# jessegrabowski/gEconpy

Hardware: AMD Instinct MI355X
Metric: solve+Kalman-logp evals/sec, Smets-Wouters n~40 T=200 (higher is better)
Workload: dtype f64; 1 GPU; sw_shaped synthetic (SURVEY 8d): n=m=40, n_state=18, n_lead=12, k=7, p=7, T_len=200, 4096 draws per GPU (BASELINE configs[2]); global_batch=4096, solver=cycle_reduction, inputs=A,B,C,D resident in HBM, parallelism=single GPU

## Files before the change

### geconpy_amd/csrc/dsge_kalman_mf.hpp

```cpp
#pragma once
#include <type_traits>

#include "dsge_kalman_nt.hpp"
#include "dsge_kalman_rec.hpp"
#include "dsge_mfma4.hpp"

namespace dsge {

template <int KT, int TM>
struct KmfSmem {
  static_assert(KT >= 1 && KT <= TM && TM <= 8, "tiles");
  static constexpr int NS = 4 * KT, NM = 4 * TM;
  static constexpr int LDK = NS + 2;
  static constexpr int NR = 8 * ((NM + 7) / 8);
  static constexpr int RP = NR / 8, PS = 10;
  static constexpr int WT = NM * LDK > NR * PS ? NM * LDK : NR * PS;
  static constexpr size_t doubles = (size_t)NM * LDK + WT + (size_t)NS * LDK + 2 * (size_t)NR * PS + 2 * NR + 4 + 44 + NR / 2 + 4;
  static constexpr size_t bytes = sizeof(double) * doubles;
};

#ifndef KMF_WAVES
#define KMF_WAVES 2
#endif
template <int KT, int TM, bool DBG, bool REC = false, int RBS = (4 * TM + 7) / 8>
__global__ __launch_bounds__(64, KMF_WAVES) void kalman_mf_kernel(
    const double* __restrict__ T, const double* __restrict__ RQR, const double* __restrict__ P0, const double* __restrict__ Z,
    int z_batched, const double* __restrict__ dvec, int d_batched, const double* __restrict__ Hdiag, int h_batched,
    const double* __restrict__ y, int batch, int m_full, int p, int T_len, FilterConv cv, double missing_fill, double steady_tol,
    double* __restrict__ logp_out, int32_t* __restrict__ status, long long* __restrict__ dbg, int rerun_only,
    int32_t* __restrict__ steady_at, const int32_t* __restrict__ order, const double* __restrict__ Rsel,
    const double* __restrict__ qdiag, int q_batched, int k_shocks, const unsigned long long* __restrict__ colmask_in,
    double* __restrict__ rec_store = nullptr) {
  using SM = KmfSmem<KT, TM>;
  using RC = KgRec<RBS>;
  static_assert(!REC || (4 * TM <= 8 * RBS && Mfma4Upper<TM>::NG * 64 <= 8 * RBS * 8 * RBS), "the record's tile holds the filter's");
  using UX = Mfma4Upper<TM>;
  using MW = Mfma4Map<KT, TM>;
  constexpr int NS = SM::NS, NM = SM::NM, LDK = SM::LDK, NR = SM::NR, RP = SM::RP, PS = SM::PS, NG = UX::NG;
  constexpr bool LEAN = NG > 5;
  extern __shared__ __attribute__((aligned(16))) double smem[];
  double* Tc = smem;
  double* Wt = Tc + NM * LDK;
  double* Vs = Wt;
  double* Pc = Wt + SM::WT;
  double* PZt = Pc + NS * LDK;
  double* Ks = PZt + NR * PS;
  double* av = Ks + NR * PS;
  double* avd = av;
  double* af = av + NR + 2;
  double* vv = af + NR + 2;
  double* dd = vv + 10;
  double* hh = dd + 8;
  double* zv = hh + 8;
  double* zvt = zv + 8;
  int* perm = (int*)(zvt + 10);
  int* zpos = perm + NR;
  constexpr int W_DUMP = (NM - 1) * LDK + LDK - 1;
  constexpr int TC_DUMP = (NM - 1) * LDK + LDK - 1;
  constexpr int PC_DUMP = (NS - 1) * LDK + LDK - 1;
  constexpr int PZ_DUMP = (NR - 1) * PS + PS - 1;
  const int lane = threadIdx.x;
  const int blk = (lane >> 2) & 3, i4 = lane & 3, kq = lane >> 4;
  const double LN2PI = 1.8378770664093453, LN2 = 0.6931471805599453;

  if (rerun_only && rerun_pass_is_empty(status, batch, order)) return;
  for (int bi = blockIdx.x; bi < batch; bi = batch) {
    const int draw = __builtin_amdgcn_readfirstlane(order ? order[bi] : bi);
    const int32_t st_in = __builtin_amdgcn_readfirstlane(status[draw]);
    if (rerun_only) {
      if (st_in != DSGE_ST_INTERNAL_RERUN) continue;
    } else if (st_in != 0) {
      if (lane == 0) logp_out[draw] = -INFINITY;
      continue;
    }
    const size_t off = (size_t)draw * m_full * m_full;
    wave_sync();
    for (int idx = lane; idx < (int)SM::doubles; idx += 64) smem[idx] = 0.0;

    const double* Zg = Z + (z_batched ? (size_t)draw * p * m_full : 0);
    bool is_state = false;
    const unsigned long long cm_in = colmask_in ? colmask_in[draw] : ~0ull;
    if (cm_in != ~0ull) {
      is_state = (lane < m_full) && ((cm_in >> lane) & 1ull);
    } else {
      const double* tcol = T + off + (lane < m_full ? lane : 0);
      for (int r0 = 0; r0 < m_full; r0 += 8) {
        double tv[8];
#pragma unroll
        for (int u = 0; u < 8; ++u) tv[u] = tcol[(size_t)(r0 + u < m_full ? r0 + u : m_full - 1) * m_full];
        __builtin_amdgcn_sched_barrier(0);
#pragma unroll
        for (int u = 0; u < 8; ++u) is_state |= (tv[u] != 0.0);
      }
      is_state = is_state && (lane < m_full);
    }
    const unsigned long long colmask = __ballot(is_state);
    unsigned long long obsmask = 0ull, used = 0ull;
    bool ok = true;
    double zrow[8];
    {
      const int zl_lane = lane < m_full ? lane : m_full - 1;
#pragma unroll
      for (int o = 0; o < 8; ++o) zrow[o] = Zg[(size_t)(o < p ? o : (p > 0 ? p - 1 : 0)) * m_full + zl_lane];
      __builtin_amdgcn_sched_barrier(0);
#pragma unroll
      for (int o = 0; o < 8; ++o) zrow[o] = (lane < m_full && o < p) ? zrow[o] : 0.0;
    }
#pragma unroll
    for (int o = 0; o < 8; ++o) {
      if (o < p) {
        const unsigned long long b = __ballot(zrow[o] != 0.0);
        if (__popcll(b) != 1 || ((used & b) != 0ull)) ok = false;
        used |= b;
        obsmask |= b;
      }
    }
    const unsigned long long extra = obsmask & ~colmask;
    const int s = __popcll(colmask);
    const int m = s + __popcll(extra);
    ok = ok && (s <= NS) && (m <= NM) && (s >= 1);
    int my_pos = -1;
    if (lane < m_full) {
      const unsigned long long below = (1ull << lane) - 1ull;
      if ((colmask >> lane) & 1ull)
        my_pos = __popcll(colmask & below);
      else if ((extra >> lane) & 1ull)
        my_pos = s + __popcll(extra & below);
      if (my_pos >= 0 && my_pos < NR) perm[my_pos] = lane;
    }
#pragma unroll
    for (int o = 0; o < 8; ++o) {
      if (o < p && zrow[o] != 0.0) {
        zpos[o] = (my_pos >= 0 && my_pos < NR) ? my_pos : 0;
        zv[o] = zrow[o];
      }
    }
    if (!ok) {
      if (lane == 0) status[draw] = DSGE_ST_INTERNAL_RERUN;
      continue;
    }
    if (rerun_only && lane == 0) status[draw] = 0;
    wave_sync();

    int rr[NG], cc[NG];
    bool inm[NG], up[NG];
    constexpr int NT_ = LEAN ? 1 : NG;
    int pcw0_[NT_], pcw1_[NT_];
    int pzw0[NG], pzw1[NG];
    double pzv0_[NT_], pzv1_[NT_];
    if (lane < 9) zvt[lane] = (lane < p) ? zv[lane] : 0.0;
#pragma unroll
    for (int g = 0; g < NG; ++g) {
      int ta, tb;
      bool live;
      UX::tile(g, blk, ta, tb, live);
      const int r = 4 * ta + kq, c = 4 * tb + i4;
      rr[g] = r;
      cc[g] = c;
      inm[g] = live && r < m && c < m;
      up[g] = live && r <= c;
      int oc = -1, orr = -1;
      double zc = 0.0, zr = 0.0;
      for (int o = 0; o < p; ++o) {
        if (zpos[o] == c) {
          oc = o;
          zc = zv[o];
        }
        if (zpos[o] == r) {
          orr = o;
          zr = zv[o];
        }
      }
      const bool w0 = up[g] && inm[g] && oc >= 0, w1 = up[g] && inm[g] && r < c && orr >= 0;
      if constexpr (LEAN) {
        pzw0[g] = ((w0 ? r * PS + oc : PZ_DUMP) << 4) | (w0 ? oc : 8);
        pzw1[g] = ((w1 ? c * PS + orr : PZ_DUMP) << 4) | (w1 ? orr : 8);
      } else {
        const bool in_pc = up[g] && c < NS;
        pcw0_[g] = in_pc ? r * LDK + c : PC_DUMP;
        pcw1_[g] = (in_pc && r < c) ? c * LDK + r : PC_DUMP;
        pzw0[g] = w0 ? r * PS + oc : PZ_DUMP;
        pzw1[g] = w1 ? c * PS + orr : PZ_DUMP;
        pzv0_[g] = zc;
        pzv1_[g] = zr;
      }
    }
    int rowa[NG], rowb[NG];
    mfma4_upper_rows<TM>(lane, rowa, rowb);
    auto pcw0 = [&](int g) {
      if constexpr (LEAN) return (up[g] && cc[g] < NS) ? rr[g] * LDK + cc[g] : PC_DUMP;
      else return pcw0_[g];
    };
    auto pcw1 = [&](int g) {
      if constexpr (LEAN) return (up[g] && cc[g] < NS && rr[g] < cc[g]) ? cc[g] * LDK + rr[g] : PC_DUMP;
      else return pcw1_[g];
    };
    wave_sync();

    auto load_T = [&]() {
      lane_loop_batched<8>(m * s, lane,
                           [&](int idx) {
                             const int r = idx / s, c = idx - r * s;
                             return T[off + (size_t)perm[r] * m_full + perm[c]];
                           },
                           [&](int idx, double v) {
                             const int r = idx / s, c = idx - r * s;
                             Tc[r * LDK + c] = v;
                           });
    };
    double Qt[NG], Pt[NG];
    if (Rsel) {
      const int kp = (k_shocks + 1) & ~1;
      const double* Rg = Rsel + (size_t)draw * m_full * k_shocks;
      for (int idx = lane; idx < m_full * k_shocks; idx += 64) {
        const int i = idx / k_shocks, c = idx - i * k_shocks;
        Wt[i * kp + c] = Rg[idx];
      }
      const double* qd = qdiag + (q_batched ? (size_t)draw * k_shocks : 0);
      wave_sync();
#pragma unroll
      for (int g = 0; g < NG; ++g) {
        const double2* ri = reinterpret_cast<const double2*>(Wt + (inm[g] ? perm[rr[g]] : 0) * kp);
        const double2* rj = reinterpret_cast<const double2*>(Wt + (inm[g] ? perm[cc[g]] : 0) * kp);
        double a0 = 0.0, a1 = 0.0;
        for (int c2 = 0; 2 * c2 < kp; ++c2) {
          const double2 ti = ri[c2], tj = rj[c2];
          a0 = fma(ti.x * tj.x, qd[2 * c2], a0);
          a1 = fma(ti.y * tj.y, (2 * c2 + 1 < k_shocks) ? qd[2 * c2 + 1] : 0.0, a1);
        }
        Qt[g] = inm[g] ? a0 + a1 : 0.0;
      }
      wave_sync();
      for (int idx = lane; idx < m_full * kp; idx += 64) Wt[idx] = 0.0;
    } else {
#pragma unroll
      for (int g = 0; g < NG; ++g) Qt[g] = inm[g] ? RQR[off + (size_t)perm[rr[g]] * m_full + perm[cc[g]]] : 0.0;
    }
#pragma unroll
    for (int g = 0; g < NG; ++g) Pt[g] = (inm[g] && P0) ? P0[off + (size_t)perm[rr[g]] * m_full + perm[cc[g]]] : 0.0;
    load_T();
    wave_sync();
#define KMF_STORE_PC()                        \
  do {                                        \
    _Pragma("unroll") for (int g = 0; g < NG; ++g) { \
      Pc[pcw0(g)] = Pt[g];                    \
      Pc[pcw1(g)] = Pt[g];                    \
    }                                         \
  } while (0)
    if (!P0) {
#pragma unroll
      for (int g = 0; g < NG; ++g) Pt[g] = Qt[g];
      bool lyap_ok = false;
      for (int itl = 0; itl < 64; ++itl) {
        wave_sync();
        KMF_STORE_PC();
        wave_sync();
        mfma4_nt<KT, KT, TM, LDK>(Pc, Tc, lane, [&](int g, double d) {
          const int at = (4 * MW::tb(g, blk) + i4) * LDK + 4 * MW::ta(g, blk) + kq;
          Wt[MW::live(g, blk) ? at : W_DUMP] = d;
        });
        using MA = Mfma4Map<TM, KT>;
        double a2r[MA::NG];
        mfma4_nn<KT, TM, KT, LDK>(Tc, Tc, lane, [&](int g, double d) { a2r[g] = d; });
        wave_sync();
        double dmax = 0.0, pmax = 0.0;
        mfma4_nt_upper_acc<KT, TM, LDK>(Tc, Wt, lane, rowa, rowb, [](int) { return 0.0; }, [&](int g, double d) {
          const double dlt = inm[g] ? d : 0.0;
          Pt[g] += dlt;
          dmax = nanmax(dmax, fabs(dlt));
          pmax = nanmax(pmax, fabs(Pt[g]));
        });
        wave_sync();
#pragma unroll
        for (int g = 0; g < MA::NG; ++g) {
          const int at = (4 * MA::ta(g, blk) + kq) * LDK + 4 * MA::tb(g, blk) + i4;
          Tc[MA::live(g, blk) ? at : TC_DUMP] = a2r[g];
        }
        dmax = wave_nanmax(dmax);
        pmax = wave_nanmax(pmax);
        if (!(dmax == dmax) || !(pmax < 1e300)) break;
        if (dmax <= 1e-17 * pmax) {
          lyap_ok = true;
          break;
        }
      }
      wave_sync();
      for (int idx = lane; idx < NM * LDK; idx += 64) Tc[idx] = 0.0;
      for (int idx = lane; idx < SM::WT; idx += 64) Wt[idx] = 0.0;
      wave_sync();
      load_T();
      if (!lyap_ok) {
        if (lane == 0) {
          status[draw] |= DSGE_ST_LYAP_FAIL;
          logp_out[draw] = -INFINITY;
        }
        continue;
      }
    }
    double* const rec_d = REC ? rec_store + (size_t)draw * RC::per_draw(T_len) : nullptr;
    int seg_src = -1;
    if constexpr (REC) {
      constexpr int RNP = 8 * RBS;
      double* p0s = rec_d + (size_t)T_len * RC::STEP;
      for (int idx = lane; idx < RNP * RNP; idx += 64) {
        const int r = idx / RNP, c = idx - r * RNP;
        if (!(r < m && c < m)) p0s[idx] = 0.0;
      }
#pragma unroll
      for (int g = 0; g < NG; ++g) {
        if (up[g] && inm[g]) {
          p0s[rr[g] * RNP + cc[g]] = Pt[g];
          p0s[cc[g] * RNP + rr[g]] = Pt[g];
        }
      }
      if (lane == 0) rec_d[RC::tail_state_off(T_len) + RC::TS_LAYOUT] = (double)(RC::LAYOUT_TILES + TM);
    }
    if (lane < 8) {
      dd[lane] = (dvec && lane < p) ? dvec[(d_batched ? (size_t)draw * p : 0) + lane] : 0.0;
      hh[lane] = (Hdiag && lane < p) ? Hdiag[(h_batched ? (size_t)draw * p : 0) + lane] : 0.0;
    }
#define KMF_STORE_PZT()                                 \
  do {                                                  \
    _Pragma("unroll") for (int g = 0; g < NG; ++g) {    \
      if constexpr (LEAN) {                             \
        PZt[pzw0[g] >> 4] = zvt[pzw0[g] & 15] * Pt[g];  \
        PZt[pzw1[g] >> 4] = zvt[pzw1[g] & 15] * Pt[g];  \
      } else {                                          \
        PZt[pzw0[g]] = pzv0_[g] * Pt[g];                \
        PZt[pzw1[g]] = pzv1_[g] * Pt[g];                \
      }                                                 \
    }                                                   \
  } while (0)
    KMF_STORE_PZT();
    const int v_zpos = (lane < p) ? zpos[lane] : 0;
    const double v_zv = (lane < p) ? zv[lane] : 0.0, v_dd = (lane < 8) ? dd[lane & 7] : 0.0;
    wave_sync();

    const int r8 = lane & 7, g8 = lane >> 3;
    const int r_zpos = (r8 < p) ? zpos[r8] : 0;
    const double r_zv = (r8 < p) ? zv[r8] : 0.0, r_dd = dd[r8], r_hh = hh[r8];
    const bool fold_a = m < NM;

    double quad_sum = 0.0, quad_comp = 0.0;
    double ld_mant = 1.0;
    int ld_exp = 0;
    int n_ll_steps = 0, n_obs_entries = 0;
    long long ph[8] = {0, 0, 0, 0, 0, 0, 0, 0};
    const long long tk_start = DBG ? clock64() : 0;
    int steady_step = -1;
    const int r8c = (r8 < p) ? r8 : (p > 0 ? p - 1 : 0);
    double yt_next = (T_len > 0) ? y[r8c] : 0.0;
    for (int t = 0; t < T_len; ++t) {
      long long tk0 = DBG ? clock64() : 0;
      const double yt = yt_next;
      yt_next = y[(size_t)((t + 1 < T_len) ? t + 1 : t) * p + r8c];
      const bool obs = (r8 < p) && (yt == yt) && (yt != missing_fill);
      const unsigned long long omask = __ballot(obs) & 0xffull;
      const int n_obs = __popcll(omask);
      double* const sg = REC ? rec_d + (size_t)t * RC::STEP : nullptr;
      if constexpr (REC) {
        if (lane < 8 * RBS) sg[RC::OFF_A + lane] = (lane < NR) ? av[lane] : 0.0;
        if (lane == 0) {
          sg[RC::OFF_SRC] = (double)t;
          sg[RC::OFF_PREV] = (double)seg_src;
        }
        seg_src = t;
      }
      double2 fr2[4], pz2[RP][4];
      double pzo[RP], avi[RP];
#pragma unroll
      for (int q2 = 0; q2 < 4; ++q2) fr2[q2] = *reinterpret_cast<const double2*>(&PZt[r_zpos * PS + 2 * q2]);
      const double a_sel = av[r_zpos];
      auto load_panel = [&]() {
#pragma unroll
        for (int ps = 0; ps < RP; ++ps) {
          const int i = g8 + 8 * ps;
#pragma unroll
          for (int q2 = 0; q2 < 4; ++q2) pz2[ps][q2] = *reinterpret_cast<const double2*>(&PZt[i * PS + 2 * q2]);
          pzo[ps] = PZt[i * PS + r8];
          avi[ps] = av[i];
        }
      };
      if constexpr (!LEAN) load_panel();
      __builtin_amdgcn_sched_barrier(0);
      bool steady = false;
      double pm = 0.0;
      if (steady_tol > 0.0) {
        double pscale = 0.0;
#pragma unroll
        for (int g = 0; g < NG; ++g) pscale = fmax(pscale, (rr[g] == cc[g]) ? fabs(Pt[g]) : 0.0);
        const unsigned hi = (unsigned)__double2hiint(pscale), lo = (unsigned)__double2loint(pscale);
        const unsigned mhi = wave_max_u32(hi);
        const unsigned mlo = wave_max_u32(hi == mhi ? lo : 0u);
        pm = __hiloint2double((int)mhi, (int)mlo);
      }
      const double c_r = obs ? r_zv : 0.0;
      const double v_r = (obs ? yt : 0.0) - (((obs || !cv.mask_d) ? r_dd : 0.0) + c_r * a_sel);
      const double dg = (r8 < p) ? ((obs ? r_hh : 0.0) + cv.jit_F) : 1.0;
      vv[lane < 8 ? lane : 8] = v_r;
      asm volatile("" ::: "memory");
      double fr[8];
#pragma unroll
      for (int q = 0; q < 8; ++q) {
        const double tq = (q & 1) ? fr2[q >> 1].y : fr2[q >> 1].x;
        const double wq = ((omask >> q) & 1ull) ? 1.0 : 0.0;
        const double f = (c_r * tq) * wq;
        fr[q] = (q == r8) ? f + dg : f;
      }
      if constexpr (REC) {
        if (lane < 8) {
#pragma unroll
          for (int q = 0; q < 8; ++q) sg[RC::OFF_F + lane * 8 + q] = fr[q];
        }
      }
      double step_mant = 1.0, inv_own = 1.0;
      int step_exp = 0;
      auto pivot = [&](auto jt) {
        constexpr int j = decltype(jt)::value;
        double rowj[8];
#pragma unroll
        for (int q = 0; q < 8; ++q) rowj[q] = readlane_f64(fr[q], j);
        double inv = __builtin_amdgcn_rcp(rowj[j]);
        inv = inv * fma(-rowj[j], inv, 2.0);
        const bool is_j = (r8 == j);
        const double ci = is_j ? 0.0 : fr[j] * inv;
#pragma unroll
        for (int q = 0; q < 8; ++q)
          if (q != j) fr[q] = fma(-ci, rowj[q], fr[q]);
        fr[j] = is_j ? 1.0 : -ci;
        inv_own = is_j ? inv : inv_own;
        int e;
        step_mant *= frexp(rowj[j], &e);
        step_exp += e;
      };
      if (p >= 7) {
        pivot(std::integral_constant<int, 0>{});
        pivot(std::integral_constant<int, 1>{});
        pivot(std::integral_constant<int, 2>{});
        pivot(std::integral_constant<int, 3>{});
        pivot(std::integral_constant<int, 4>{});
        pivot(std::integral_constant<int, 5>{});
        pivot(std::integral_constant<int, 6>{});
        if (p > 7) pivot(std::integral_constant<int, 7>{});
      } else {
        pivot(std::integral_constant<int, 0>{});
        if (p > 1) pivot(std::integral_constant<int, 1>{});
        if (p > 2) pivot(std::integral_constant<int, 2>{});
        if (p > 3) pivot(std::integral_constant<int, 3>{});
        if (p > 4) pivot(std::integral_constant<int, 4>{});
        if (p > 5) pivot(std::integral_constant<int, 5>{});
      }
      if constexpr (REC) {
        if (lane < 8) {
#pragma unroll
          for (int q = 0; q < 8; ++q) sg[RC::OFF_FI + lane * 8 + q] = fr[q] * inv_own;
        }
      }
      {
        const double2* vv2 = reinterpret_cast<const double2*>(vv);
        double w0 = 0.0, w1 = 0.0;
#pragma unroll
        for (int q2 = 0; q2 < 4; ++q2) {
          const double2 vq = vv2[q2];
          w0 = fma(fr[2 * q2], vq.x, w0);
          w1 = fma(fr[2 * q2 + 1], vq.y, w1);
        }
        {
          const bool any = n_obs > 0;
          const double yk = ((lane < 8) ? (v_r * inv_own) * (w0 + w1) : 0.0) - quad_comp;
          const double tk = quad_sum + yk;
          quad_comp = any ? (tk - quad_sum) - yk : quad_comp;
          quad_sum = any ? tk : quad_sum;
          int e;
          const double lm = frexp(ld_mant * step_mant, &e);
          ld_mant = any ? lm : ld_mant;
          ld_exp += any ? e + step_exp : 0;
          n_ll_steps += any ? 1 : 0;
          n_obs_entries += n_obs;
        }
      }
      if constexpr (DBG) {
        const long long tk1 = clock64();
        ph[0] += tk1 - tk0;
        tk0 = tk1;
      }
      if constexpr (LEAN) load_panel();
#pragma unroll
      for (int ps = 0; ps < RP; ++ps) {
        const int i = g8 + 8 * ps;
        double k0 = 0.0, k1 = 0.0;
#pragma unroll
        for (int q2 = 0; q2 < 4; ++q2) {
          k0 = fma(pz2[ps][q2].x, fr[2 * q2], k0);
          k1 = fma(pz2[ps][q2].y, fr[2 * q2 + 1], k1);
        }
        const double kk = obs ? (k0 + k1) * inv_own : 0.0;
        Ks[i * PS + r8] = kk;
        Vs[i * PS + r8] = -fma(cv.jit_V, kk, obs ? pzo[ps] : 0.0);
        double part = kk * v_r;
        part += dpp_move_f64<0xB1, 0xf>(part);
        part += dpp_move_f64<0x4E, 0xf>(part);
        part += dpp_move_f64<0x141, 0xf>(part);
        af[(r8 == 0) ? i : NR] = avi[ps] + part;
      }
      wave_sync();
      if constexpr (REC) {
        for (int idx = lane; idx < 8 * RBS * 8; idx += 64) sg[RC::OFF_K + idx] = ((idx >> 3) < NR) ? Ks[(idx >> 3) * PS + (idx & 7)] : 0.0;
      }
      if constexpr (DBG) {
        const long long tk1 = clock64();
        ph[1] += tk1 - tk0;
        tk0 = tk1;
      }
      {
        double dmax = 0.0;
        mfma4_nt_upper_acc<2, TM, PS>(Ks, Vs, lane, rowa, rowb, [&](int g) { return Pt[g]; },
                                      [&](int g, double d) {
                                        const double pn = inm[g] ? d + ((rr[g] == cc[g]) ? cv.jit_P : 0.0) : 0.0;
                                        Pt[g] = pn;
                                      });
        if constexpr (REC) {
#pragma unroll
          for (int g = 0; g < NG; ++g) sg[(size_t)g * 64 + lane] = Pt[g];
        }
        if (steady_tol > 0.0) {
          if constexpr (!LEAN) {
            double oldv[NG];
#pragma unroll
            for (int g = 0; g < NG; ++g) oldv[g] = *reinterpret_cast<const volatile double*>(&Pc[pcw0(g)]);
#pragma unroll
            for (int g = 0; g < NG; ++g) dmax = fmax(dmax, (pcw0(g) != PC_DUMP) ? fabs(Pt[g] - oldv[g]) : 0.0);
          } else {
#pragma unroll
            for (int g = 0; g < NG; ++g) {
              const int at = pcw0(g);
              const double old = *reinterpret_cast<const volatile double*>(&Pc[at]);
              dmax = fmax(dmax, (at != PC_DUMP) ? fabs(Pt[g] - old) : 0.0);
            }
          }
          steady = (t > 0) && (__ballot(!(dmax <= steady_tol * pm)) == 0ull);
        }
        KMF_STORE_PC();
      }
      double af_l = 0.0;
      if (fold_a) {
        af_l = af[lane < NR ? lane : 0];
      } else if (lane < m) {
        const double2* trow2 = reinterpret_cast<const double2*>(Tc + lane * LDK);
        const double2* af2 = reinterpret_cast<const double2*>(af);
        double s0 = 0.0, s1 = 0.0;
        for (int kk = 0; 2 * kk < s; ++kk) {
          const double2 tv2 = trow2[kk], fv = af2[kk];
          s0 = fma(tv2.x, fv.x, s0);
          s1 = fma(tv2.y, fv.y, s1);
        }
        av[lane] = s0 + s1;
      }
      wave_sync();
      if constexpr (DBG) {
        const long long tk1 = clock64();
        ph[2] += tk1 - tk0;
        tk0 = tk1;
      }
      mfma4_nt<KT, KT, TM, LDK>(Pc, Tc, lane, [&](int g, double d) {
        const int at = (4 * MW::tb(g, blk) + i4) * LDK + 4 * MW::ta(g, blk) + kq;
        Wt[MW::live(g, blk) ? at : W_DUMP] = d;
      });
      Wt[(fold_a && lane < NS) ? m * LDK + lane : W_DUMP] = af_l;
      wave_sync();
      if constexpr (DBG) {
        const long long tk1 = clock64();
        ph[3] += tk1 - tk0;
        tk0 = tk1;
      }
      mfma4_nt_upper_acc<KT, TM, LDK>(Tc, Wt, lane, rowa, rowb, [&](int g) { return Qt[g]; },
                                      [&](int g, double d) {
                                        const bool is_mean = fold_a && cc[g] == m && rr[g] < m && up[g];
                                        avd[is_mean ? rr[g] : NR] = is_mean ? d : 0.0;
                                        Pt[g] = inm[g] ? d : 0.0;
                                      });
      KMF_STORE_PZT();
      wave_sync();
      if constexpr (DBG) {
        const long long tk1 = clock64();
        ph[4] += tk1 - tk0;
        tk0 = tk1;
      }
      if (!steady) continue;
      if (steady_step < 0) steady_step = t + 1;
      {
        double trow[NS], finv_row[8], kr_ss[8];
        double av_reg = (lane < m) ? av[lane] : 0.0;
#pragma unroll
        for (int kk = 0; kk < NS; ++kk) trow[kk] = (lane < NM) ? Tc[lane * LDK + kk] : 0.0;
#pragma unroll
        for (int q = 0; q < 8; ++q) {
          finv_row[q] = (lane < 8) ? fr[q] * inv_own : 0.0;
          kr_ss[q] = (lane < m) ? Ks[lane * PS + q] : 0.0;
        }
        while (t + 1 < T_len) {
          const double yt_s = yt_next;
          const bool obs_s = (lane < p) && (yt_s == yt_s) && (yt_s != missing_fill);
          if (__ballot(obs_s) != omask) break;
          ++t;
          yt_next = y[(size_t)((t + 1 < T_len) ? t + 1 : t) * p + r8c];
          if constexpr (REC) {
            double* sgs = rec_d + (size_t)t * RC::STEP;
            if (lane < 8 * RBS) sgs[RC::OFF_A + lane] = av_reg;
            if (lane == 0) sgs[RC::OFF_SRC] = (double)seg_src;
          }
          const double av_sel = __shfl(av_reg, v_zpos, 64);
          double v_s = 0.0;
          if (lane < p) v_s = (obs_s ? yt_s : 0.0) - (((obs_s || !cv.mask_d) ? v_dd : 0.0) + (obs_s ? 1.0 : 0.0) * (v_zv * av_sel));
          double vsc[8];
#pragma unroll
          for (int o = 0; o < 8; ++o) vsc[o] = readlane_f64(v_s, o);
          double w0 = 0.0, w1 = 0.0, a0 = av_reg, a1 = 0.0;
#pragma unroll
          for (int o = 0; o < 8; o += 2) {
            w0 = fma(finv_row[o], vsc[o], w0);
            w1 = fma(finv_row[o + 1], vsc[o + 1], w1);
            a0 = fma(kr_ss[o], vsc[o], a0);
            a1 = fma(kr_ss[o + 1], vsc[o + 1], a1);
          }
          if (n_obs > 0) {
            const double yk = v_s * (w0 + w1) - quad_comp;
            const double tk = quad_sum + yk;
            quad_comp = (tk - quad_sum) - yk;
            quad_sum = tk;
            int e;
            ld_mant = frexp(ld_mant * step_mant, &e);
            ld_exp += e + step_exp;
            ++n_ll_steps;
            n_obs_entries += n_obs;
          }
          const double afi = a0 + a1;
          double s0 = 0.0, s1 = 0.0;
#pragma unroll
          for (int kk = 0; kk < NS; kk += 2) {
            s0 = fma(trow[kk], readlane_f64(afi, kk), s0);
            s1 = fma(trow[kk + 1], readlane_f64(afi, kk + 1), s1);
          }
          av_reg = (lane < m) ? s0 + s1 : 0.0;
          if constexpr (DBG) ++ph[6];
        }
        if (lane < m) av[lane] = av_reg;
      }
      wave_sync();
      if constexpr (DBG) ph[5] += clock64() - tk0;
    }
#undef KMF_STORE_PZT
#undef KMF_STORE_PC
    if (DBG && dbg && draw == 0 && lane == 0) {
      ph[7] = clock64() - tk_start;
      for (int k = 0; k < 8; ++k) dbg[k] = ph[k];
    }
    const double quad_total = wave_sum_dpp(quad_sum - quad_comp);
    if (lane == 0) {
      const double logdet = log(ld_mant) + (double)ld_exp * LN2;
      const double ll = -0.5 * (cv.ll_terms(n_ll_steps, n_obs_entries, p) * LN2PI + logdet + quad_total);
      logp_out[draw] = ll;
      if (steady_at) steady_at[draw] = steady_step;
      if (!((ll == ll) && (fabs(ll) < 1.797e308))) status[draw] |= DSGE_ST_FILTER_NONFINITE;
    }
  }
}

}
```

Measured before the change: 3.226 million evals/s.

## Hoist old-P loads early and specialize steady-state loop on state count

Loads the previous covariance values for the steady-state check before the sched barrier, not after the update, so their LDS latency overlaps other work (non-lean, non-record path). The lean path uses an explicit LDS address-space volatile pointer in place of a generic one. The steady-state loop is rewritten as a lambda templated on the column count, which skips the last two state columns when they are unused and batches readlanes in groups of six with sched barriers. The per-lane obs predicate and d term are precomputed outside the loop. This trades register pressure from holding oldv early for shorter loop iterations.

```diff
diff --git a/geconpy_amd/csrc/dsge_kalman_mf.hpp b/geconpy_amd/csrc/dsge_kalman_mf.hpp
--- a/geconpy_amd/csrc/dsge_kalman_mf.hpp
+++ b/geconpy_amd/csrc/dsge_kalman_mf.hpp
@@ -38,6 +38,7 @@
   using MW = Mfma4Map<KT, TM>;
   constexpr int NS = SM::NS, NM = SM::NM, LDK = SM::LDK, NR = SM::NR, RP = SM::RP, PS = SM::PS, NG = UX::NG;
   constexpr bool LEAN = NG > 5;
+  constexpr bool OLD_EARLY = !LEAN && !REC;
   extern __shared__ __attribute__((aligned(16))) double smem[];
   double* Tc = smem;
   double* Wt = Tc + NM * LDK;
@@ -382,6 +383,11 @@
         }
       };
       if constexpr (!LEAN) load_panel();
+      double oldv[OLD_EARLY ? NG : 1];
+      if constexpr (OLD_EARLY) {
+#pragma unroll
+        for (int g = 0; g < NG; ++g) oldv[g] = Pc[pcw0(g)];
+      }
       __builtin_amdgcn_sched_barrier(0);
       bool steady = false;
       double pm = 0.0;
@@ -524,17 +530,15 @@
           for (int g = 0; g < NG; ++g) sg[(size_t)g * 64 + lane] = Pt[g];
         }
         if (steady_tol > 0.0) {
-          if constexpr (!LEAN) {
-            double oldv[NG];
-#pragma unroll
-            for (int g = 0; g < NG; ++g) oldv[g] = *reinterpret_cast<const volatile double*>(&Pc[pcw0(g)]);
+          if constexpr (OLD_EARLY) {
 #pragma unroll
             for (int g = 0; g < NG; ++g) dmax = fmax(dmax, (pcw0(g) != PC_DUMP) ? fabs(Pt[g] - oldv[g]) : 0.0);
           } else {
+            using LdsCVD = const volatile __attribute__((address_space(3))) double*;
 #pragma unroll
             for (int g = 0; g < NG; ++g) {
               const int at = pcw0(g);
-              const double old = *reinterpret_cast<const volatile double*>(&Pc[at]);
+              const double old = *(LdsCVD)(&Pc[at]);
               dmax = fmax(dmax, (at != PC_DUMP) ? fabs(Pt[g] - old) : 0.0);
             }
           }
@@ -598,52 +602,69 @@
           finv_row[q] = (lane < 8) ? fr[q] * inv_own : 0.0;
           kr_ss[q] = (lane < m) ? Ks[lane * PS + q] : 0.0;
         }
-        while (t + 1 < T_len) {
-          const double yt_s = yt_next;
-          const bool obs_s = (lane < p) && (yt_s == yt_s) && (yt_s != missing_fill);
-          if (__ballot(obs_s) != omask) break;
-          ++t;
-          yt_next = y[(size_t)((t + 1 < T_len) ? t + 1 : t) * p + r8c];
-          if constexpr (REC) {
-            double* sgs = rec_d + (size_t)t * RC::STEP;
-            if (lane < 8 * RBS) sgs[RC::OFF_A + lane] = av_reg;
-            if (lane == 0) sgs[RC::OFF_SRC] = (double)seg_src;
+        const bool obs_l = (lane < p) && ((omask >> lane) & 1ull);
+        const double d_l = (obs_l || !cv.mask_d) ? v_dd : 0.0, one_l = obs_l ? 1.0 : 0.0;
+        const unsigned long long pbits = (1ull << p) - 1ull;
+        auto steady_loop = [&](auto nc_tag) {
+          constexpr int NC = decltype(nc_tag)::value;
+          while (t + 1 < T_len) {
+            const double yt_s = yt_next;
+            if ((__builtin_amdgcn_ballot_w64(yt_s == yt_s) & __builtin_amdgcn_ballot_w64(yt_s != missing_fill) & pbits) != omask) break;
+            ++t;
+            yt_next = y[(size_t)((t + 1 < T_len) ? t + 1 : t) * p + r8c];
+            if constexpr (REC) {
+              double* sgs = rec_d + (size_t)t * RC::STEP;
+              if (lane < 8 * RBS) sgs[RC::OFF_A + lane] = av_reg;
+              if (lane == 0) sgs[RC::OFF_SRC] = (double)seg_src;
+            }
+            const double av_sel = __shfl(av_reg, v_zpos, 64);
+            const double v_s = (lane < p) ? (obs_l ? yt_s : 0.0) - (d_l + one_l * (v_zv * av_sel)) : 0.0;
+            double vsc[8];
+#pragma unroll
+            for (int o = 0; o < 8; ++o) vsc[o] = readlane_f64(v_s, o);
+            double w0 = 0.0, w1 = 0.0, a0 = av_reg, a1 = 0.0;
+#pragma unroll
+            for (int o = 0; o < 8; o += 2) {
+              w0 = fma(finv_row[o], vsc[o], w0);
+              w1 = fma(finv_row[o + 1], vsc[o + 1], w1);
+              a0 = fma(kr_ss[o], vsc[o], a0);
+              a1 = fma(kr_ss[o + 1], vsc[o + 1], a1);
+            }
+            if (n_obs > 0) {
+              const double yk = v_s * (w0 + w1) - quad_comp;
+              const double tk = quad_sum + yk;
+              quad_comp = (tk - quad_sum) - yk;
+              quad_sum = tk;
+              int e;
+              ld_mant = frexp(ld_mant * step_mant, &e);
+              ld_exp += e + step_exp;
+              ++n_ll_steps;
+              n_obs_entries += n_obs;
+            }
+            const double afi = a0 + a1;
+            double s0 = 0.0, s1 = 0.0;
+#pragma unroll
+            for (int b0 = 0; b0 < NC; b0 += 6) {
+              const int b1 = (NC - b0 <= 8) ? NC : b0 + 6;
+              double afs[8];
+#pragma unroll
+              for (int kk = b0; kk < b1; ++kk) afs[kk - b0] = readlane_f64(afi, kk);
+#pragma unroll
+              for (int kk = b0; kk < b1; kk += 2) {
+                s0 = fma(trow[kk], afs[kk - b0], s0);
+                s1 = fma(trow[kk + 1], afs[kk + 1 - b0], s1);
+              }
+              if (b1 == NC) break;
+              __builtin_amdgcn_sched_barrier(0);
+            }
+            av_reg = s0 + s1;
+            if constexpr (DBG) ++ph[6];
           }
-          const double av_sel = __shfl(av_reg, v_zpos, 64);
-          double v_s = 0.0;
-          if (lane < p) v_s = (obs_s ? yt_s : 0.0) - (((obs_s || !cv.mask_d) ? v_dd : 0.0) + (obs_s ? 1.0 : 0.0) * (v_zv * av_sel));
-          double vsc[8];
-#pragma unroll
-          for (int o = 0; o < 8; ++o) vsc[o] = readlane_f64(v_s, o);
-          double w0 = 0.0, w1 = 0.0, a0 = av_reg, a1 = 0.0;
-#pragma unroll
-          for (int o = 0; o < 8; o += 2) {
-            w0 = fma(finv_row[o], vsc[o], w0);
-            w1 = fma(finv_row[o + 1], vsc[o + 1], w1);
-            a0 = fma(kr_ss[o], vsc[o], a0);
-            a1 = fma(kr_ss[o + 1], vsc[o + 1], a1);
-          }
-          if (n_obs > 0) {
-            const double yk = v_s * (w0 + w1) - quad_comp;
-            const double tk = quad_sum + yk;
-            quad_comp = (tk - quad_sum) - yk;
-            quad_sum = tk;
-            int e;
-            ld_mant = frexp(ld_mant * step_mant, &e);
-            ld_exp += e + step_exp;
-            ++n_ll_steps;
-            n_obs_entries += n_obs;
-          }
-          const double afi = a0 + a1;
-          double s0 = 0.0, s1 = 0.0;
-#pragma unroll
-          for (int kk = 0; kk < NS; kk += 2) {
-            s0 = fma(trow[kk], readlane_f64(afi, kk), s0);
-            s1 = fma(trow[kk + 1], readlane_f64(afi, kk + 1), s1);
-          }
-          av_reg = (lane < m) ? s0 + s1 : 0.0;
-          if constexpr (DBG) ++ph[6];
-        }
+        };
+        if (s <= NS - 2)
+          steady_loop(std::integral_constant<int, NS - 2>{});
+        else
+          steady_loop(std::integral_constant<int, NS>{});
         if (lane < m) av[lane] = av_reg;
       }
       wave_sync();
```

Result: faster. 3.311 million evals/s (median of 6 runs) (+2.6%).
